# OpenVisualCloud/SVT-VP9

Measured on AMD Instinct MI355X. Metric: hot-path frames/sec (+ Mpixels/sec): block-level DSP path (picture analysis + ME + inter prediction from reconstructed references + DCT/quant/recon + deblock + reference padding), 3840x2160p60 yuv420p enc-mode 8; no mode decision, no entropy coding -- not encoded frames, higher is better.
Workload: dtype u8

## Files before the change

svt-vp9_amd/csrc/intra_kernel.hip:

```cpp
#include <hip/hip_runtime.h>
#include "tq_core.h"
#include "encdec_core.h"
#include "intra_pred.h"
#include <stdlib.h>

namespace {

struct intra_pic_dev {
    const uint8_t *src[3];
    uint8_t       *pred[3];
    uint8_t       *rec[3];
    int32_t        src_stride[2], pred_stride[2], rec_stride[2];
    const svt_lf_mode_info *mi;
    int32_t        mi_stride, mi_rows, mi_cols, sb_cols, sb_rows, width, height;
    const svt_quant_tables *qtabs;
    const int16_t *iscan;
    uint32_t       iscan_off[16];
    int16_t       *qcoeff, *dqcoeff;
    uint16_t      *eob_map;
    uint8_t       *nz;
    int32_t       *sync;
    int32_t       *status;
    int32_t        mixed;
};

#ifdef INTRA_FENCES
#define INTRA_WT false
#define INTRA_LD(p) (*(p))
#else
#define INTRA_WT true
#define INTRA_LD(p) __hip_atomic_load((p), __ATOMIC_RELAXED, __HIP_MEMORY_SCOPE_AGENT)
#endif
#ifdef INTRA_PROF
__device__ unsigned long long g_intra_fine[8];
#define IPF(k) do { if (lane == 0) { const unsigned long long n_ = __builtin_amdgcn_s_memtime(); atomicAdd(&g_intra_fine[k], n_ - ipf_t); ipf_t = n_; } } while (0)
#else
#define IPF(k) ((void)0)
#endif
template <int N>
__device__ __forceinline__ int intra_block(const intra_pic_dev &P, int plane, int x0, int y0, int mode, int sb, int32_t *tile, uint8_t *edge, int have_right = 0) {
    const int lane = (int)threadIdx.x, c = plane ? 1 : 0;
    const int rs = P.rec_stride[c];
    uint8_t  *rp = P.rec[plane];
    const int have_left = x0 > 0, have_top = y0 > 0;
    const bool active = lane < N;
    const int  i = lane % N;
#ifdef INTRA_PROF
    unsigned long long ipf_t = __builtin_amdgcn_s_memtime();
#endif
    uint32_t   srow[N / 4], prow[N / 4];
    constexpr uintptr_t AM = N >= 16 ? 15 : N - 1;
    {
        const uint8_t *sp = P.src[plane] + (size_t)(y0 + i) * P.src_stride[c] + x0;
        _Pragma("unroll") for (int q = 0; q < N / 4; q++) srow[q] = 0u;
        if (active) row_load<N>(sp, ((uintptr_t)sp & AM) == 0, srow);
    }
    {
        const int j = lane & 31;
        if (lane < 32) {
            if (j < N) edge[32 - (j + 1)] = have_left ? INTRA_LD(&rp[(size_t)(y0 + j) * rs + x0 - 1]) : (uint8_t)129;
        } else {
            if (j < N) {
                const uint8_t a = have_top ? INTRA_LD(&rp[(size_t)(y0 - 1) * rs + x0 + j]) : (uint8_t)127;
                edge[32 + 1 + j] = a;
                if (N == 4 && have_right) edge[32 + 1 + N + j] = have_top ? INTRA_LD(&rp[(size_t)(y0 - 1) * rs + x0 + N + j]) : (uint8_t)127;
                else if (j == N - 1) { _Pragma("unroll") for (int q = 0; q < N; q++) edge[32 + 1 + N + q] = a; }
            }
        }
        if (lane == 0) edge[32] = have_top ? (have_left ? INTRA_LD(&rp[(size_t)(y0 - 1) * rs + x0 - 1]) : (uint8_t)129) : (uint8_t)127;
    }
    __syncthreads();
    IPF(0);
    intra_pred_row<N>(edge, mode, i, have_left, have_top, prow);
    {
        if (active && P.pred[plane]) {
            uint8_t *pp = P.pred[plane] + (size_t)(y0 + i) * P.pred_stride[c] + x0;
            row_store<N>(pp, ((uintptr_t)pp & AM) == 0, prow);
        }
    }
    IPF(1);
    svt_tq_block k;
    k.src_off = k.pred_off = 0;
    k.recon_off = (uint32_t)y0 * (uint32_t)rs + (uint32_t)x0;
    k.coeff_off = (uint32_t)sb * SVT_SB_COEFFS + (plane == 0 ? 0u : plane == 1 ? 4096u : 5120u) + svt_zorder4((x0 & (plane ? 31 : 63)) >> 2, (y0 & (plane ? 31 : 63)) >> 2) * 16u;
    k.tx_size = (uint8_t)txcfg<N>::size;
    k.tx_type = (uint8_t)((plane == 0 && N < 32) ? intra_tx_type(mode) : 0);
    k.iscan_off = P.iscan_off[k.tx_size * 4 + k.tx_type];
    k.src_stride = k.pred_stride = 0; k.recon_stride = (uint16_t)rs;
    k.qtab = (uint8_t)c; k.do_recon = 1; k.partial32 = 0; k.pad_[0] = 0;
    const int pw4 = (plane ? P.width >> 1 : P.width) >> 2, w4 = P.width >> 2, h4 = P.height >> 2;
    const int eo = plane == 0 ? 0 : w4 * h4 + (plane == 2 ? (w4 >> 1) * (h4 >> 1) : 0);
    int32_t *t = tile + (lane / N) * (N * (N + 1));
    const int eob = tq_block_body<N, false, false, INTRA_WT>(k, active, i, t, srow, prow, P.qtabs, P.iscan, P.qcoeff, P.dqcoeff,
                                                   P.eob_map + eo + (y0 >> 2) * pw4 + (x0 >> 2), nullptr, nullptr, nullptr, nullptr, nullptr, rp);
    IPF(2);
    __builtin_amdgcn_fence(__ATOMIC_SEQ_CST, "workgroup");
    __syncthreads();
    IPF(3);
    return __builtin_amdgcn_readfirstlane(eob);
}

#ifndef INTRA_WAVES_PER_EU
#define INTRA_WAVES_PER_EU 4
#endif
#ifdef INTRA_NUM_VGPR
__attribute__((amdgpu_num_vgpr(INTRA_NUM_VGPR)))
#endif
__global__ __launch_bounds__(64) __attribute__((amdgpu_waves_per_eu(INTRA_WAVES_PER_EU, INTRA_WAVES_PER_EU))) void svt_intra_kernel(const intra_pic_dev P) {
    __shared__ int32_t tile[2 * 32 * 33];
    __shared__ uint8_t edge[128];
    __shared__ int32_t s_ticket;
    const int lane = (int)threadIdx.x, c_cols = (P.width + 15) >> 4, c_rows = (P.height + 15) >> 4, n_cell = c_cols * c_rows;
    const int n_diag = c_rows + c_cols - 1;
    __builtin_amdgcn_s_setprio(3);
#ifdef INTRA_PROF
  unsigned long long pf[5] = {0, 0, 0, 0, 0}, pf_n = 0;
#endif
  for (;;) {
    __syncthreads();
    if (lane == 0) s_ticket = atomicAdd(&P.sync[0], 1);
    __syncthreads();
#ifdef INTRA_PROF
    if (s_ticket >= 3 * n_cell) { if (lane == 0 && blockIdx.x == 0) printf("[intra-fine] refs %llu predict %llu tq %llu drain %llu (summed over all workgroups so far)\n", g_intra_fine[0], g_intra_fine[1], g_intra_fine[2], g_intra_fine[3]);
      if (lane == 0 && blockIdx.x < 2) printf("[intra-prof] wg %d cells %llu: ticket+map %llu wait %llu work %llu drain %llu publish %llu (100 MHz ticks)\n", (int)blockIdx.x, pf_n, pf[0], pf[1], pf[2], pf[3], pf[4]); break; }
    unsigned long long pt0 = __builtin_amdgcn_s_memtime();
#else
    if (s_ticket >= 3 * n_cell) break;
#endif
    const int ticket = s_ticket, plane = ticket % 3;
    const int n = ticket / 3, m = c_rows < c_cols ? c_rows : c_cols, M = c_rows < c_cols ? c_cols : c_rows;
    int lo = 0, hi = n_diag;
    auto count = [&](int d) -> int {
        const int a = d < m ? d : m;
        int       t = a * (a + 1) / 2;
        if (d > m) { const int fl = (d < M ? d : M) - m; t += fl * m; }
        if (d > M) { const int k = d - M; t += k * m - k * (k + 1) / 2; }
        return t;
    };
    while (hi - lo > 1) { const int mid = (lo + hi) >> 1; if (count(mid) <= n) lo = mid; else hi = mid; }
    const int d = lo, r_lo = d - (c_cols - 1) > 0 ? d - (c_cols - 1) : 0;
    const int cr = r_lo + (n - count(d)), cc = d - cr;
    const int cell = cr * c_cols + cc;
    int32_t  *done = P.sync + 2 + plane * n_cell;
    const int  br = cr & ~1, bc = cc & ~1;
    const int  ub_r = br * 2, ub_c = bc * 2;
    const svt_lf_mode_info b0 = P.mi[ub_r * P.mi_stride + ub_c];
    const bool big = b0.sb_type == 9 && !(b0.is_inter && P.mixed) && ub_r + 4 <= P.mi_rows && ub_c + 4 <= P.mi_cols;
    if (big && !(cr == br && cc == bc + 1)) continue;
    const int ur0 = cr * 2, uc0 = cc * 2;
#ifdef INTRA_PROF
    unsigned long long pt1 = __builtin_amdgcn_s_memtime();
#endif
    if (lane == 0) {
        const int wl_r = big ? br + 1 : cr, wl_c = (big ? bc : cc) - 1;
        const int wa_r = (big ? br : cr) - 1, wa_c = big ? bc + 1 : cc;
        if (wl_c >= 0) while (__hip_atomic_load(&done[wl_r * c_cols + wl_c], __ATOMIC_RELAXED, __HIP_MEMORY_SCOPE_AGENT) == 0) __builtin_amdgcn_s_sleep(2);
        if (wa_r >= 0) while (__hip_atomic_load(&done[wa_r * c_cols + wa_c], __ATOMIC_RELAXED, __HIP_MEMORY_SCOPE_AGENT) == 0) __builtin_amdgcn_s_sleep(2);
    }
    __syncthreads();
#ifdef INTRA_FENCES
    __builtin_amdgcn_fence(__ATOMIC_ACQUIRE, "agent");
#endif
#ifdef INTRA_PROF
    unsigned long long pt2 = __builtin_amdgcn_s_memtime();
#endif
    const int nu = big ? 1 : 4, u_r = big ? ub_r : ur0, u_c = big ? ub_c : uc0;
    for (int z = 0; z < nu; z++) {
        const int r = (z >> 1) & 1, c = z & 1;
        const int ur = u_r + r, uc = u_c + c;
        if (ur >= P.mi_rows || uc >= P.mi_cols) continue;
        const svt_lf_mode_info b = P.mi[ur * P.mi_stride + uc];
        const int sub = b.sb_type == 0;
        const int w8 = b.sb_type == 3 || sub ? 1 : b.sb_type == 6 ? 2 : b.sb_type == 9 ? 4 : 0;
        if (b.is_inter && P.mixed) continue;
        if (w8 == 0 || b.is_inter) { if (lane == 0) atomicOr(P.status, 1); continue; }
        if ((ur % w8) || (uc % w8)) continue;
        if (w8 == 4 && !big) { if (lane == 0) atomicOr(P.status, 1); continue; }
        const int mode = plane ? b.pad_[2] : b.pad_[1];
        if (ur + w8 > P.mi_rows || uc + w8 > P.mi_cols || b.tx_size != (sub ? 0 : w8 == 1 ? 1 : w8 == 2 ? 2 : 3) || (!sub && mode > 9) || b.pad_[2] > 9) {
            if (lane == 0) atomicOr(P.status, 1);
            continue;
        }
        const int sb = (ur >> 3) * P.sb_cols + (uc >> 3);
        const int x0 = plane ? uc * 4 : uc * 8, y0 = plane ? ur * 4 : ur * 8, nn = plane ? w8 * 4 : w8 * 8;
        int eob;
        if (sub && plane == 0) {
            const int m4 = (int)b.pad_[1] | (int)b.pad_[0] << 8;
            eob = 0;
            for (int q4 = 0; q4 < 4; q4++) {
                const int mq = (m4 >> (4 * q4)) & 15;
                if (mq > 9) { if (lane == 0) atomicOr(P.status, 1); continue; }
                eob |= intra_block<4>(P, 0, x0 + 4 * (q4 & 1), y0 + 4 * (q4 >> 1), mq, sb, tile, edge, !(q4 & 1));
            }
        }
        else if (nn == 32) eob = intra_block<32>(P, plane, x0, y0, mode, sb, tile, edge);
        else if (nn == 16) eob = intra_block<16>(P, plane, x0, y0, mode, sb, tile, edge);
        else if (nn == 8) eob = intra_block<8>(P, plane, x0, y0, mode, sb, tile, edge);
        else eob = intra_block<4>(P, plane, x0, y0, mode, sb, tile, edge);
        if (eob && lane == 0) P.nz[ur * P.mi_stride + uc] = 1;
    }
#ifdef INTRA_PROF
    unsigned long long pt3 = __builtin_amdgcn_s_memtime();
#endif
#ifdef INTRA_FENCES
    __builtin_amdgcn_fence(__ATOMIC_RELEASE, "agent");
    __syncthreads();
#else
    asm volatile("s_waitcnt vmcnt(0)" ::: "memory");
    __syncthreads();
#endif
#ifdef INTRA_PROF
    unsigned long long pt4 = __builtin_amdgcn_s_memtime();
#endif
    if (lane == 0) {
        if (big) {
            _Pragma("unroll") for (int k = 0; k < 4; k++) {
                const int rr = br + (k >> 1), c2 = bc + (k & 1);
                if (rr < c_rows && c2 < c_cols) __hip_atomic_store(&done[rr * c_cols + c2], 1, __ATOMIC_RELAXED, __HIP_MEMORY_SCOPE_AGENT);
            }
        } else __hip_atomic_store(&done[cell], 1, __ATOMIC_RELAXED, __HIP_MEMORY_SCOPE_AGENT);
    }
#ifdef INTRA_PROF
    { const unsigned long long pt5 = __builtin_amdgcn_s_memtime(); pf[0] += pt1 - pt0; pf[1] += pt2 - pt1; pf[2] += pt3 - pt2; pf[3] += pt4 - pt3; pf[4] += pt5 - pt4; pf_n++; }
#endif
  }
}

__global__ __launch_bounds__(256) void svt_md_intra_default_kernel(svt_lf_mode_info *mi, int mi_stride, int mi_rows, int mi_cols, int filter_level) {
    const int u = (int)(blockIdx.x * blockDim.x + threadIdx.x);
    if (u >= mi_rows * mi_cols) return;
    const int r = u / mi_cols, c = u % mi_cols;
    const int fit16 = (r & ~1) + 2 <= mi_rows && (c & ~1) + 2 <= mi_cols;
    svt_lf_mode_info m;
    m.sb_type = fit16 ? 6 : 3; m.tx_size = fit16 ? 2 : 1; m.skip = 0; m.is_inter = 0; m.filter_level = (uint8_t)filter_level;
    m.pad_[0] = m.pad_[1] = m.pad_[2] = 0;
    mi[r * mi_stride + c] = m;
}

}

int32_t svt_intra_launch(svt_hip_ctx *ctx, const svt_encdec_picture *p, int32_t width, int32_t height, int32_t mi_stride, const svt_quant_tables *d_qtabs,
                         const int16_t *d_iscan, const uint32_t iscan_off[16], int32_t *d_sync, int32_t *d_status, int32_t mixed) {
    intra_pic_dev P;
    memset(&P, 0, sizeof P);
    P.src[0] = p->src.y; P.src[1] = p->src.u; P.src[2] = p->src.v;
    P.pred[0] = p->pred.y; P.pred[1] = p->pred.u; P.pred[2] = p->pred.v;
    P.rec[0] = p->recon.y; P.rec[1] = p->recon.u; P.rec[2] = p->recon.v;
    P.src_stride[0] = p->src.y_stride; P.src_stride[1] = p->src.uv_stride;
    P.pred_stride[0] = p->pred.y_stride; P.pred_stride[1] = p->pred.uv_stride;
    P.rec_stride[0] = p->recon.y_stride; P.rec_stride[1] = p->recon.uv_stride;
    P.mi = p->d_lf_mi; P.mi_stride = mi_stride; P.mi_rows = height >> 3; P.mi_cols = width >> 3;
    P.sb_cols = (width + 63) >> 6; P.sb_rows = (height + 63) >> 6; P.width = width; P.height = height;
    P.qtabs = d_qtabs; P.iscan = d_iscan;
    for (int i = 0; i < 16; i++) P.iscan_off[i] = iscan_off[i];
    P.qcoeff = p->d_qcoeff; P.dqcoeff = p->d_dqcoeff; P.eob_map = p->d_eob_map; P.nz = p->d_nz; P.sync = d_sync; P.status = d_status; P.mixed = mixed;
    const int n_cell = ((width + 15) >> 4) * ((height + 15) >> 4);
    HIP_TRY(hipMemsetAsync(d_sync, 0, (size_t)(2 + 3 * n_cell) * sizeof(int32_t), ctx->stream));
    static const int wg_per_cu = [] { const char *e = getenv("SVT_HIP_INTRA_WG_PER_CU"); return e && atoi(e) > 0 ? atoi(e) : 2; }();
    static const int wg_cap = [] { const char *e = getenv("SVT_HIP_INTRA_WGS"); return e && atoi(e) > 0 ? atoi(e) : 0; }();
    int grid = ctx->cu_count * wg_per_cu;
    const int cap = ctx->intra_wgs > 0 ? ctx->intra_wgs : wg_cap;
    if (cap && grid > cap) grid = cap;
    if (grid > 3 * n_cell) grid = 3 * n_cell;
    hipLaunchKernelGGL(svt_intra_kernel, dim3(grid), dim3(64), 0, ctx->stream, P);
    HIP_TRY(hipGetLastError());
    return SVT_HIP_OK;
}

int32_t svt_md_intra_default_launch(svt_hip_ctx *ctx, svt_lf_mode_info *d_lf_mi, int32_t mi_stride, int32_t mi_rows, int32_t mi_cols, int32_t filter_level) {
    hipLaunchKernelGGL(svt_md_intra_default_kernel, dim3((mi_rows * mi_cols + 255) / 256), dim3(256), 0, ctx->stream, d_lf_mi, mi_stride, mi_rows, mi_cols, filter_level);
    HIP_TRY(hipGetLastError());
    return SVT_HIP_OK;
}
```

Measured before the change: 6276.

## Pack four independent intra workers as waves into one workgroup

The intra kernel now launches workgroups of four waves. Each wave acts as an independent worker with its own LDS slice for the tile and edge buffers. Workgroup barriers become wave-level syncs (tq_block_sync), and tickets are broadcast with readfirstlane instead of through shared memory. The aim is fewer workgroup dispatches and cheaper per-cell synchronisation, while keeping the total worker count the same. The risk is that the four waves are co-scheduled on one CU with a larger LDS footprint, which may hurt distribution across CUs.

```diff
diff --git a/svt-vp9_amd/csrc/intra_kernel.hip b/svt-vp9_amd/csrc/intra_kernel.hip
--- a/svt-vp9_amd/csrc/intra_kernel.hip
+++ b/svt-vp9_amd/csrc/intra_kernel.hip
@@ -37,9 +37,14 @@
 #else
 #define IPF(k) ((void)0)
 #endif
+#define INTRA_TILE_DW  (2 * 32 * 33)
+#define INTRA_SLICE_DW (INTRA_TILE_DW + 128 / 4)
+#define INTRA_W        4
 template <int N>
-__device__ __forceinline__ int intra_block(const intra_pic_dev &P, int plane, int x0, int y0, int mode, int sb, int32_t *tile, uint8_t *edge, int have_right = 0) {
-    const int lane = (int)threadIdx.x, c = plane ? 1 : 0;
+__device__ __forceinline__ int intra_block(const intra_pic_dev &P, int plane, int x0, int y0, int mode, int sb, int32_t *lds, int have_right = 0) {
+    const int lane = (int)__lane_id(), c = plane ? 1 : 0;
+    int32_t *const tile = lds + __builtin_amdgcn_readfirstlane((int)threadIdx.x >> 6) * INTRA_SLICE_DW;
+    uint8_t *const edge = (uint8_t *)(tile + INTRA_TILE_DW);
     const int rs = P.rec_stride[c];
     uint8_t  *rp = P.rec[plane];
     const int have_left = x0 > 0, have_top = y0 > 0;
@@ -69,7 +74,7 @@
         }
         if (lane == 0) edge[32] = have_top ? (have_left ? INTRA_LD(&rp[(size_t)(y0 - 1) * rs + x0 - 1]) : (uint8_t)129) : (uint8_t)127;
     }
-    __syncthreads();
+    tq_block_sync();
     IPF(0);
     intra_pred_row<N>(edge, mode, i, have_left, have_top, prow);
     {
@@ -95,7 +100,7 @@
                                                    P.eob_map + eo + (y0 >> 2) * pw4 + (x0 >> 2), nullptr, nullptr, nullptr, nullptr, nullptr, rp);
     IPF(2);
     __builtin_amdgcn_fence(__ATOMIC_SEQ_CST, "workgroup");
-    __syncthreads();
+    tq_block_sync();
     IPF(3);
     return __builtin_amdgcn_readfirstlane(eob);
 }
@@ -106,28 +111,31 @@
 #ifdef INTRA_NUM_VGPR
 __attribute__((amdgpu_num_vgpr(INTRA_NUM_VGPR)))
 #endif
-__global__ __launch_bounds__(64) __attribute__((amdgpu_waves_per_eu(INTRA_WAVES_PER_EU, INTRA_WAVES_PER_EU))) void svt_intra_kernel(const intra_pic_dev P) {
-    __shared__ int32_t tile[2 * 32 * 33];
-    __shared__ uint8_t edge[128];
-    __shared__ int32_t s_ticket;
-    const int lane = (int)threadIdx.x, c_cols = (P.width + 15) >> 4, c_rows = (P.height + 15) >> 4, n_cell = c_cols * c_rows;
+__global__ __launch_bounds__(64 * INTRA_W) __attribute__((amdgpu_waves_per_eu(INTRA_WAVES_PER_EU, INTRA_WAVES_PER_EU))) void svt_intra_kernel(const intra_pic_dev P, const int n_workers) {
+    constexpr int W = INTRA_W;
+    __shared__ int32_t s_lds[W * INTRA_SLICE_DW];
+    const int wave = __builtin_amdgcn_readfirstlane((int)threadIdx.x >> 6);
+    if ((int)blockIdx.x * W + wave >= n_workers) return;
+    const int lane = (int)__lane_id(), c_cols = (P.width + 15) >> 4, c_rows = (P.height + 15) >> 4, n_cell = c_cols * c_rows;
     const int n_diag = c_rows + c_cols - 1;
     __builtin_amdgcn_s_setprio(3);
 #ifdef INTRA_PROF
   unsigned long long pf[5] = {0, 0, 0, 0, 0}, pf_n = 0;
+  const int worker = (int)blockIdx.x * W + wave;
 #endif
   for (;;) {
-    __syncthreads();
-    if (lane == 0) s_ticket = atomicAdd(&P.sync[0], 1);
-    __syncthreads();
-#ifdef INTRA_PROF
-    if (s_ticket >= 3 * n_cell) { if (lane == 0 && blockIdx.x == 0) printf("[intra-fine] refs %llu predict %llu tq %llu drain %llu (summed over all workgroups so far)\n", g_intra_fine[0], g_intra_fine[1], g_intra_fine[2], g_intra_fine[3]);
-      if (lane == 0 && blockIdx.x < 2) printf("[intra-prof] wg %d cells %llu: ticket+map %llu wait %llu work %llu drain %llu publish %llu (100 MHz ticks)\n", (int)blockIdx.x, pf_n, pf[0], pf[1], pf[2], pf[3], pf[4]); break; }
+    tq_block_sync();
+    int drawn = 0;
+    if (lane == 0) drawn = atomicAdd(&P.sync[0], 1);
+    const int ticket = __builtin_amdgcn_readfirstlane(drawn);
+#ifdef INTRA_PROF
+    if (ticket >= 3 * n_cell) { if (lane == 0 && worker == 0) printf("[intra-fine] refs %llu predict %llu tq %llu drain %llu (summed over all workers so far)\n", g_intra_fine[0], g_intra_fine[1], g_intra_fine[2], g_intra_fine[3]);
+      if (lane == 0 && worker < 2) printf("[intra-prof] worker %d cells %llu: ticket+map %llu wait %llu work %llu drain %llu publish %llu (100 MHz ticks)\n", worker, pf_n, pf[0], pf[1], pf[2], pf[3], pf[4]); break; }
     unsigned long long pt0 = __builtin_amdgcn_s_memtime();
 #else
-    if (s_ticket >= 3 * n_cell) break;
-#endif
-    const int ticket = s_ticket, plane = ticket % 3;
+    if (ticket >= 3 * n_cell) break;
+#endif
+    const int plane = ticket % 3;
     const int n = ticket / 3, m = c_rows < c_cols ? c_rows : c_cols, M = c_rows < c_cols ? c_cols : c_rows;
     int lo = 0, hi = n_diag;
     auto count = [&](int d) -> int {
@@ -157,7 +165,7 @@
         if (wl_c >= 0) while (__hip_atomic_load(&done[wl_r * c_cols + wl_c], __ATOMIC_RELAXED, __HIP_MEMORY_SCOPE_AGENT) == 0) __builtin_amdgcn_s_sleep(2);
         if (wa_r >= 0) while (__hip_atomic_load(&done[wa_r * c_cols + wa_c], __ATOMIC_RELAXED, __HIP_MEMORY_SCOPE_AGENT) == 0) __builtin_amdgcn_s_sleep(2);
     }
-    __syncthreads();
+    tq_block_sync();
 #ifdef INTRA_FENCES
     __builtin_amdgcn_fence(__ATOMIC_ACQUIRE, "agent");
 #endif
@@ -190,13 +198,13 @@
             for (int q4 = 0; q4 < 4; q4++) {
                 const int mq = (m4 >> (4 * q4)) & 15;
                 if (mq > 9) { if (lane == 0) atomicOr(P.status, 1); continue; }
-                eob |= intra_block<4>(P, 0, x0 + 4 * (q4 & 1), y0 + 4 * (q4 >> 1), mq, sb, tile, edge, !(q4 & 1));
+                eob |= intra_block<4>(P, 0, x0 + 4 * (q4 & 1), y0 + 4 * (q4 >> 1), mq, sb, s_lds, !(q4 & 1));
             }
         }
-        else if (nn == 32) eob = intra_block<32>(P, plane, x0, y0, mode, sb, tile, edge);
-        else if (nn == 16) eob = intra_block<16>(P, plane, x0, y0, mode, sb, tile, edge);
-        else if (nn == 8) eob = intra_block<8>(P, plane, x0, y0, mode, sb, tile, edge);
-        else eob = intra_block<4>(P, plane, x0, y0, mode, sb, tile, edge);
+        else if (nn == 32) eob = intra_block<32>(P, plane, x0, y0, mode, sb, s_lds);
+        else if (nn == 16) eob = intra_block<16>(P, plane, x0, y0, mode, sb, s_lds);
+        else if (nn == 8) eob = intra_block<8>(P, plane, x0, y0, mode, sb, s_lds);
+        else eob = intra_block<4>(P, plane, x0, y0, mode, sb, s_lds);
         if (eob && lane == 0) P.nz[ur * P.mi_stride + uc] = 1;
     }
 #ifdef INTRA_PROF
@@ -204,10 +212,10 @@
 #endif
 #ifdef INTRA_FENCES
     __builtin_amdgcn_fence(__ATOMIC_RELEASE, "agent");
-    __syncthreads();
+    tq_block_sync();
 #else
     asm volatile("s_waitcnt vmcnt(0)" ::: "memory");
-    __syncthreads();
+    tq_block_sync();
 #endif
 #ifdef INTRA_PROF
     unsigned long long pt4 = __builtin_amdgcn_s_memtime();
@@ -256,13 +264,13 @@
     P.qcoeff = p->d_qcoeff; P.dqcoeff = p->d_dqcoeff; P.eob_map = p->d_eob_map; P.nz = p->d_nz; P.sync = d_sync; P.status = d_status; P.mixed = mixed;
     const int n_cell = ((width + 15) >> 4) * ((height + 15) >> 4);
     HIP_TRY(hipMemsetAsync(d_sync, 0, (size_t)(2 + 3 * n_cell) * sizeof(int32_t), ctx->stream));
-    static const int wg_per_cu = [] { const char *e = getenv("SVT_HIP_INTRA_WG_PER_CU"); return e && atoi(e) > 0 ? atoi(e) : 2; }();
-    static const int wg_cap = [] { const char *e = getenv("SVT_HIP_INTRA_WGS"); return e && atoi(e) > 0 ? atoi(e) : 0; }();
-    int grid = ctx->cu_count * wg_per_cu;
-    const int cap = ctx->intra_wgs > 0 ? ctx->intra_wgs : wg_cap;
-    if (cap && grid > cap) grid = cap;
-    if (grid > 3 * n_cell) grid = 3 * n_cell;
-    hipLaunchKernelGGL(svt_intra_kernel, dim3(grid), dim3(64), 0, ctx->stream, P);
+    static const int wk_per_cu = [] { const char *e = getenv("SVT_HIP_INTRA_WG_PER_CU"); return e && atoi(e) > 0 ? atoi(e) : 2; }();
+    static const int wk_cap = [] { const char *e = getenv("SVT_HIP_INTRA_WGS"); return e && atoi(e) > 0 ? atoi(e) : 0; }();
+    int workers = ctx->cu_count * wk_per_cu;
+    const int cap = ctx->intra_wgs > 0 ? ctx->intra_wgs : wk_cap;
+    if (cap && workers > cap) workers = cap;
+    if (workers > 3 * n_cell) workers = 3 * n_cell;
+    hipLaunchKernelGGL(svt_intra_kernel, dim3((workers + INTRA_W - 1) / INTRA_W), dim3(64 * INTRA_W), 0, ctx->stream, P, workers);
     HIP_TRY(hipGetLastError());
     return SVT_HIP_OK;
 }
```

New measurement: 6533 (median of 6 runs). 4.1% higher.
